# selbouhaddani/PPLS

Measured on AMD Instinct MI355X. Metric: EM iterations/sec + log-lik rel-err vs CPU ref, n=1e6 p=q=2000 r=5, higher is better.
Workload: dtype f64

## Files before the change

### include/ppls_debug.h

```cpp
#ifndef PPLS_AMD_PPLS_DEBUG_H
#define PPLS_AMD_PPLS_DEBUG_H

#include "ppls.h"

#ifdef __cplusplus
extern "C" {
#endif

int ppls_sweep_timing(ppls_ctx* ctx, double* total_ms, int64_t* launches, int reset);
int ppls_sweep_balance(ppls_ctx* ctx, double* w8, int64_t* bounds, int cap, int* n_bounds);
int ppls_comm_info(ppls_ctx* ctx, int* nranks, int* rank, double* allreduce_ms, int64_t* allreduce_calls,
                   int reset);
int ppls_xprod_info(ppls_ctx* ctx, int r, int* ready, int64_t* bytes_per_pass, double* flops, int* rows_per_wave);
int ppls_xprod_setup_times(ppls_ctx* ctx, double* gram_ms, double* allreduce_ms, double* total_ms);
int ppls_xprod_tile_timing(ppls_ctx* ctx, int reps, double* ms);
int ppls_xprod_stats(ppls_ctx* ctx, const ppls_theta* th, int r, double* stats);
int ppls_sweep_info(ppls_ctx* ctx, int r, int64_t* bytes_per_sweep, int* variant, int* grid);
int ppls_sweep_kernel(ppls_ctx* ctx, int r, char* buf, int len);
int ppls_gram_int8(ppls_ctx* ctx, int which, double* G, int* nmod, int* L, double* ms);
int ppls_gram_shifts(ppls_ctx* ctx, int* shift, int P, int* count);
int ppls_oz_residue_host(double x, int shift, int l, int* r);
int ppls_oz_crt_host(const int* r, int nmod, double* out);
int ppls_oz_modulus(int l);
int ppls_gram_info(ppls_ctx* ctx, int* int8_used, int* nmod, int* L, double* ms);
int ppls_meta_info(ppls_ctx* ctx, int* path);
int ppls_gram(ppls_ctx* ctx, int xory, int nsplit, double* G, double* ms);
int ppls_spd_inverse(ppls_ctx* ctx, const double* A, int p, int a, int method, double* out, int* info, double* ms);
int ppls_philox4x32_10(ppls_ctx* ctx, const uint32_t* ctr, int64_t count, uint64_t key, uint32_t* out);

#define PPLS_FTRACE_LEN 48
int ppls_finalize_trace(ppls_ctx* ctx, int64_t* stamps, double* tick_ns);
#define PPLS_STRACE_MAX_WG 4096
int ppls_sweep_trace(ppls_ctx* ctx, int64_t* stamps, int cap, int* n, double* tick_ns);
int ppls_cv_timing(ppls_ctx* ctx, double* out6, int reset);

int ppls_xprod_get(ppls_ctx* ctx, double* S, int* P, int* ldx);

int ppls_scale_timing(ppls_ctx* ctx, double* ms3, double* bytes3);

// ... 7 lines not shown
```

### ppls_amd/_lib.py

```python
from __future__ import annotations

import ctypes as ct
import os

import numpy as np

_HERE = os.path.dirname(os.path.abspath(__file__))
LIB_PATH = os.path.join(_HERE, "libppls_amd.so")

PPLS_OK = 0
PPLS_ORTH_SVD = 0
PPLS_ORTH_QR = 1
PPLS_LAYOUT_COLMAJOR = 0
PPLS_LAYOUT_ROWMAJOR = 1

_dp = ct.POINTER(ct.c_double)


class PplsTheta(ct.Structure):
    _fields_ = [("W", _dp), ("C", _dp), ("B", _dp), ("sigT", _dp),
                ("sigE", ct.c_double), ("sigF", ct.c_double), ("sigH", ct.c_double)]


class PplsExpect(ct.Structure):
# ... 81 lines not shown
    "ppls_comm_info": (ct.c_int, [ct.c_void_p, ct.POINTER(ct.c_int), ct.POINTER(ct.c_int), _dp,
                                  ct.POINTER(ct.c_int64), ct.c_int]),
    "ppls_finalize_trace": (ct.c_int, [ct.c_void_p, ct.POINTER(ct.c_int64), _dp]),
    "ppls_sweep_trace": (ct.c_int, [ct.c_void_p, ct.POINTER(ct.c_int64), ct.c_int, ct.POINTER(ct.c_int), _dp]),
    "ppls_sweep_info": (ct.c_int, [ct.c_void_p, ct.c_int, ct.POINTER(ct.c_int64), ct.POINTER(ct.c_int),
                                   ct.POINTER(ct.c_int)]),
    "ppls_sweep_kernel": (ct.c_int, [ct.c_void_p, ct.c_int, ct.c_char_p, ct.c_int]),
    "ppls_meta_info": (ct.c_int, [ct.c_void_p, ct.POINTER(ct.c_int)]),
    "ppls_gram_int8": (ct.c_int, [ct.c_void_p, ct.c_int, _dp, ct.POINTER(ct.c_int), ct.POINTER(ct.c_int), _dp]),
    "ppls_oz_residue_host": (ct.c_int, [ct.c_double, ct.c_int, ct.c_int, ct.POINTER(ct.c_int)]),
    "ppls_oz_crt_host": (ct.c_int, [ct.POINTER(ct.c_int), ct.c_int, _dp]),
    "ppls_oz_modulus": (ct.c_int, [ct.c_int]),
    "ppls_gram_info": (ct.c_int, [ct.c_void_p, ct.POINTER(ct.c_int), ct.POINTER(ct.c_int), ct.POINTER(ct.c_int),
                                  _dp]),
    "ppls_gram_shifts": (ct.c_int, [ct.c_void_p, ct.POINTER(ct.c_int), ct.c_int, ct.POINTER(ct.c_int)]),
    "ppls_finalize_host": (ct.c_int, [_dp, _dp, _dp, ct.c_double, ct.c_double, ct.c_double, ct.c_int,
                                      ct.c_int, ct.c_int, ct.POINTER(PplsTheta), ct.c_int,
                                      ct.POINTER(PplsTheta), ct.POINTER(PplsExpect), _dp]),
    "ppls_mu_coefficients": (ct.c_int, [ct.POINTER(PplsTheta), ct.c_int, _dp]),
    "ppls_set_data_from": (ct.c_int, [ct.c_void_p, ct.c_void_p, _i64p, ct.c_int64, ct.c_int64]),
    "ppls_xprod_downdate": (ct.c_int, [ct.c_void_p, ct.c_void_p, _i64p, ct.c_int64]),
    "ppls_predict": (ct.c_int, [ct.c_void_p, _dp, _dp, _dp, ct.c_int, ct.c_int, _dp, ct.c_int64, ct.c_int, _dp]),
    "ppls_heldout_sse": (ct.c_int, [ct.c_void_p, _dp, _dp, _dp, ct.c_int, _i64p, ct.c_int64, _dp]),
    "ppls_cv_ppls": (ct.c_int, [ct.c_void_p, ct.c_int, ct.c_int, ct.POINTER(ct.c_int32), _i64p, ct.c_int,
                                ct.c_double, ct.c_int, ct.POINTER(PplsTheta), _dp, ct.POINTER(ct.c_int)]),
    "ppls_cv_timing": (ct.c_int, [ct.c_void_p, _dp, ct.c_int]),
    "ppls_scale_data": (ct.c_int, [ct.c_void_p, ct.c_int, ct.c_int]),
    "ppls_get_scaling": (ct.c_int, [ct.c_void_p, _dp, _dp]),
    "ppls_scale_timing": (ct.c_int, [ct.c_void_p, _dp, _dp]),
    "ppls_xprod_get": (ct.c_int, [ct.c_void_p, _dp, ct.POINTER(ct.c_int), ct.POINTER(ct.c_int)]),
# ... 113 lines not shown
```

### ppls_amd/api.py

```python
from __future__ import annotations

import ctypes as ct
import itertools
import math
import time
import warnings

import numpy as np

from . import _lib
from ._lib import Expect, PplsError, Theta, dptr


def pop_rows(pop_sizes, row0, n_local):
    sizes = np.asarray(pop_sizes, dtype=np.int64)
    ends = np.cumsum(sizes)
    begins = ends - sizes
    lo, hi = int(row0), int(row0) + int(n_local)
    local = np.clip(np.minimum(ends, hi) - np.maximum(begins, lo), 0, None).astype(np.int64)
    return np.ascontiguousarray(local), np.ascontiguousarray(sizes)


class Context:

# ... 419 lines not shown
        nm, L, ms = ct.c_int(), ct.c_int(), np.zeros(4)
        self._chk(self._L.ppls_gram_int8(self.h, int(which), dptr(G), ct.byref(nm), ct.byref(L), dptr(ms)))
        return G, dict(nmod=nm.value, L=L.value, ms=ms.tolist(), shift=self.gram_shifts())

    def gram_shifts(self):
        k = ct.c_int()
        self._chk(self._L.ppls_gram_shifts(self.h, None, 0, ct.byref(k)))
        out = (ct.c_int * max(k.value, 1))()
        self._chk(self._L.ppls_gram_shifts(self.h, out, k.value, ct.byref(k)))
        return np.array(out[:k.value], dtype=np.int64)

    def gram_info(self):
        u, nm, L, ms = ct.c_int(), ct.c_int(), ct.c_int(), np.zeros(4)
        self._chk(self._L.ppls_gram_info(self.h, ct.byref(u), ct.byref(nm), ct.byref(L), dptr(ms)))
        return dict(int8=bool(u.value), nmod=nm.value, L=L.value, ms=ms.tolist())

    def spd_inverse(self, A, method=1):
        A = np.asarray(A, dtype=np.float64)
        one = A.ndim == 2
        A3 = A[None] if one else A
        a, p = A3.shape[0], A3.shape[1]
        Af = np.ascontiguousarray(np.transpose(A3, (0, 2, 1)))
        out = np.empty_like(Af)
        info = (ct.c_int * a)()
        ms = ct.c_double()
        self._chk(self._L.ppls_spd_inverse(self.h, dptr(Af), int(p), int(a), int(method), dptr(out), info,
                                            ct.byref(ms)))
        inv = np.transpose(out, (0, 2, 1))
        return (inv[0] if one else inv), np.array(list(info)), ms.value

# ... 969 lines not shown
```

### ppls_amd/csrc/ppls_capi.cpp

```cpp
#include <hip/hip_runtime.h>
#include <rccl/rccl.h>
#include <rocblas/rocblas.h>
#include <rocsolver/rocsolver.h>

#include <algorithm>
#include <chrono>
#include <cmath>
#include <cstdarg>
#include <cstdio>
#include <cstring>
#include <string>
#include <utility>
#include <vector>

#include "../../include/ppls.h"
#include "../../include/ppls_debug.h"
#include "ppls_kernels.h"
#include "ppls_math.h"
#include "ppls_cv.h"
#include "ppls_scale.h"
#include "ppls_cvstream.h"
#include "ppls_stream.h"
#include "ppls_xprod.h"

// ... 61 lines not shown
  int bal_grid = -1;
  double bal_w[8] = {1, 1, 1, 1, 1, 1, 1, 1};
  int64_t* bal_bounds = nullptr;
  double* coefs = nullptr;
  double* scratch = nullptr;
  size_t scratch_bytes = 0;
  int* stop_d = nullptr;
  int* stop_mirror = nullptr;
  int* stop_mirror_dev = nullptr;
  const int* sweep_stop = nullptr;
  double stop_atol = 0.0;
  int em_r = 0, em_cur = 0, em_iter = 0;
  bool em_active = false;
  int xprod = 0;
  int xprod_rw = 0;
  int gram_int8 = 0;
  int oz_used = 0, oz_nmod = 0, oz_L = 0;
  std::vector<int> oz_shift;
  double oz_ms[4] = {0, 0, 0, 0};
  int8_t* oz_planes = nullptr;
  uint8_t* oz_res = nullptr;
  size_t oz_planes_len = 0, oz_res_len = 0;
  bool xp_ready = false;
  bool xp_active = false;
  bool xp_pending_gram = false;
  int xprod_fuse = 1;
  bool xp_explicit = false;
  int meta_path = 0;
  int meta_device = 1;
  int vorth = 8;
  double* xp_S = nullptr;
// ... 605 lines not shown
  if (!part_in) dfree(part);
  if (e != hipSuccess) return fail(c, PPLS_E_HIP, "MFMA Gram: %s", hipGetErrorString(e));
  return PPLS_OK;
}

bool oz_held(const ppls_ctx* c) { return c->oz_planes || c->oz_res; }

void oz_free(ppls_ctx* c) {
  dfree(c->oz_planes);
  dfree(c->oz_res);
  c->oz_planes = nullptr;
  c->oz_res = nullptr;
  c->oz_planes_len = c->oz_res_len = 0;
}

int gram_run_oz(ppls_ctx* c, const GramShape& g, int64_t n, double* G, float* ms) {
  const int P = g.p, Pp = (P + 255) / 256 * 256;
  const int64_t nkb = (n + PPLS_OZ_KS - 1) / PPLS_OZ_KS;
  const int dtype = c->dtype;
  struct Bufs {
    double* part = nullptr;
    double* st = nullptr;
    int* shift = nullptr;
    hipEvent_t ev[5] = {nullptr, nullptr, nullptr, nullptr, nullptr};
    ~Bufs() {
      dfree(part); dfree(st); dfree(shift);
      for (auto e : ev) if (e) (void)hipEventDestroy(e);
    }
  } b;
  int rc;
  const int chunks = (int)std::max<int64_t>(1, std::min<int64_t>(256, n / 2048));
  if ((rc = dalloc(c, &b.part, (size_t)chunks * 2 * Pp)) || (rc = dalloc(c, &b.st, (size_t)2 * Pp)) ||
      (rc = dalloc(c, &b.shift, (size_t)Pp)))
    return rc;
  for (auto& e : b.ev) HIPCHK(c, hipEventCreate(&e));
  HIPCHK(c, hipEventRecord(b.ev[0], c->stream));
  HIPCHK(c, ppls_launch_oz_colstats(g.X, g.ldx, g.xcols, g.xreal, g.Y, g.ldy, g.yreal, dtype, Pp, n, chunks, b.part,
                                    b.st, c->stream));
  std::vector<double> st((size_t)2 * Pp);
  HIPCHK(c, hipMemcpyAsync(st.data(), b.st, sizeof(double) * st.size(), hipMemcpyDeviceToHost, c->stream));
  HIPCHK(c, hipStreamSynchronize(c->stream));
  auto live = [&](int j) { return j < g.xreal || (j >= g.xcols && j - g.xcols < g.yreal); };
  int L = 55;
  std::vector<int> shift((size_t)Pp, 0);
  double qmax = 0.0;
  for (int j = 0; j < P; ++j) {
    if (!live(j) || !(st[(size_t)j] > 0.0)) continue;
    int ex = 0;
    (void)std::frexp(st[(size_t)j], &ex);
    const double cj = std::max(1.0, std::ldexp(1.0, ex) * std::sqrt((double)n / st[(size_t)Pp + j]));
    const int Lj = 53 + (int)std::ceil(std::log2(cj)) + 2;
    L = std::max(L, Lj);
    shift[(size_t)j] = Lj - ex;
    const double q = std::ldexp(std::sqrt(st[(size_t)Pp + j]), Lj - ex) + 0.5 * std::sqrt((double)n);
    qmax = std::max(qmax, q * q);
  }
  c->oz_L = L;
  c->oz_shift.assign(shift.begin(), shift.begin() + P);
  if (L > 62) return 1;
  const double need = std::log2(std::max(qmax, 1.0)) + 1.0 + 1e-7;
  double bits = 0.0;
  int nmod = 0;
  while (nmod < PPLS_OZ_MAXMOD && bits < need) bits += std::log2((double)ppls_oz_modulus(nmod++));
  if (bits < need) return 1;
  nmod = std::max(nmod, 12);
  c->oz_nmod = nmod;
  const int T = Pp / 256, ntiles = T * (T + 1) / 2, nsplit = ppls_oz_splits(nkb);
  const int64_t pstride = nkb * Pp * PPLS_OZ_KS;
  const size_t need_planes = (size_t)nmod * pstride, need_res = (size_t)nmod * nsplit * ntiles * 65536;
  if (need_planes > c->oz_planes_len || need_res > c->oz_res_len) {
    HIPCHK(c, hipStreamSynchronize(c->stream));
    oz_free(c);
    size_t fr = 0, tot = 0;
    if (hipMemGetInfo(&fr, &tot) != hipSuccess) return 1;
    const double want = (double)need_planes + (double)need_res;
    if (want > (double)fr - std::max(1073741824.0, 0.05 * (double)fr)) return 1;
    if (dalloc(c, &c->oz_planes, need_planes) || dalloc(c, &c->oz_res, need_res)) {
      c->err.clear();
      oz_free(c);
      return 1;
    }
    c->oz_planes_len = need_planes;
    c->oz_res_len = need_res;
  }
  int8_t* planes = c->oz_planes;
  uint8_t* res = c->oz_res;
  HIPCHK(c, hipMemcpyAsync(b.shift, shift.data(), sizeof(int) * Pp, hipMemcpyHostToDevice, c->stream));
  HIPCHK(c, ppls_launch_oz_residues(g.X, g.ldx, g.xcols, g.xreal, g.Y, g.ldy, g.yreal, dtype, Pp, n, nkb, b.shift,
                                    nmod, planes, pstride, c->stream));
  HIPCHK(c, hipEventRecord(b.ev[1], c->stream));
  HIPCHK(c, ppls_launch_oz_syrk(planes, pstride, Pp, nkb, nmod, res, c->stream));
  HIPCHK(c, hipEventRecord(b.ev[2], c->stream));
  HIPCHK(c, ppls_launch_oz_finish(res, nmod, nsplit, Pp, g.xcols, g.xreal, g.yreal, P, b.shift, G, c->stream));
  HIPCHK(c, hipEventRecord(b.ev[3], c->stream));
  HIPCHK(c, hipStreamSynchronize(c->stream));
  float t01 = 0.f, t12 = 0.f, t23 = 0.f, t03 = 0.f;
  HIPCHK(c, hipEventElapsedTime(&t01, b.ev[0], b.ev[1]));
  HIPCHK(c, hipEventElapsedTime(&t12, b.ev[1], b.ev[2]));
  HIPCHK(c, hipEventElapsedTime(&t23, b.ev[2], b.ev[3]));
  HIPCHK(c, hipEventElapsedTime(&t03, b.ev[0], b.ev[3]));
  c->oz_ms[0] = t01;
  c->oz_ms[1] = t12;
  c->oz_ms[2] = t23;
  c->oz_ms[3] = t03;
  if (ms) *ms = t03;
  return PPLS_OK;
}

int gram_run_s(ppls_ctx* c, const GramShape& g, int64_t n, double* G, float* ms, double* part) {
  c->oz_used = 0;
  if (c->gram_int8) {
    const int rc = gram_run_oz(c, g, n, G, ms);
    if (rc == PPLS_OK) {
      c->oz_used = 1;
      return PPLS_OK;
    }
    if (rc < 0) return rc;
  }
  return gram_run(c, g, n, 0, G, ms, part);
}

int xprod_setup(ppls_ctx* c);
bool xprod_choose(ppls_ctx* c, int max_steps, int r);

int64_t xprod_rows(const ppls_ctx* c) { return (c->n_total + c->nranks - 1) / c->nranks; }

double xprod_bytes(ppls_ctx* c) {
  const GramShape g = gram_shape(c, true, 0);
  const double PP = (double)g.p * g.p;
  return 8.0 * PP + 8.0 * (double)ppls_gram_part_doubles(g.p, gram_nsplit(c, g, xprod_rows(c), 0)) +
         16.0 * g.p * PPLS_RMAX;
}
// ... 63 lines not shown
  return PPLS_OK;
}

bool xprod_choose(ppls_ctx* c, int max_steps, int r) {
  if (c->st_state == 2) return true;
  if (c->xprod == 0) return false;
  if (c->xprod == 1) return true;
  if (!c->xp_ready && xprod_bytes(c) > c->mem_free_min - std::max(1073741824.0, 0.05 * c->mem_free_min))
    return false;
  const double P = (double)(c->ldx + c->ldy);
  const double n = (double)((c->n_total + c->nranks - 1) / c->nranks);
  const double esz = c->dtype ? 4.0 : 8.0;
  const bool split = c->sweep_mode != 3 && !c->dtype && ppls_split_supported(r, c->ldx, c->ldy) > 0;
  const double t_sweep = (split ? 1.0 : 2.0) * esz * n * P / 6.5e12 + 5e-6;
  const double t_pass = 8.0 * P * P / 6.5e12 + 5e-6;
  const double gram_rate = c->gram_int8 ? 1.0e14 : 55e12;
  const double t_setup = c->xp_ready ? 0.0 : n * P * P / gram_rate + (c->nranks > 1 ? 16.0 * P * P / 100e9 : 0.0);
  return ((double)max_steps + 1.0) * (t_sweep - t_pass) > t_setup;
}

int xprod_stats(ppls_ctx* c, int r, int slot, bool fuse) {
  int rc;
  const int P = c->ldx + c->ldy;
  if (!c->xp_ready && (rc = xprod_setup(c))) return rc;
  if (!c->xp_M) {
    if ((rc = dalloc(c, &c->xp_M, (size_t)P * 2 * PPLS_RMAX))) return rc;
  }
  hipEvent_t e0, e1;
  if ((rc = timing_pair(c, &e0, &e1))) return rc;
  if (e0) HIPCHK(c, hipEventRecord(e0, c->stream));
  const int rw = ppls_xprod_tile_rows(P, r, c->xprod_rw, c->num_cus);
// ... 56 lines not shown
  c->st_fq.clear();
  c->st_fq_len.clear();
  c->st_cap = c->st_cm_len = c->st_part_len = c->st_colpart_len = c->st_gbuf_len = 0;
  c->st_state = 0;
  c->st_failed = false;
}

void fold_free(ppls_ctx* c) {
  dfree(c->st_fS);
  c->st_nfolds = 0;
  c->st_sel = -1;
  c->st_fN.clear();
  c->st_fmean_h.clear();
}

void xprod_free(ppls_ctx* c) {
  if (c->st_state) {
    stream_release(c);
    c->have_data = false;
    c->em_active = false;
  }
  c->xp_ready = false;
  c->xp_explicit = false;
  c->xp_active = false;
  dfree(c->xp_S);
  dfree(c->xp_M);
  fold_free(c);
}

int compute_ssq(ppls_ctx* c) {
  int rc;
  xprod_free(c);

  const int nb = 1024;
  const int nred = 2 + c->nranks;
  if ((rc = dalloc(c, &c->scratch, (size_t)nb + nred))) return rc;
  HIPCHK(c, hipMemsetAsync(c->ssq, 0, 2 * sizeof(double), c->stream));
  if (c->n_local > 0 && c->dtype) {
    HIPCHK(c, ppls_launch_sumsq_f32((const float*)c->X, c->n_local * c->ldx, c->scratch, nb, c->ssq, c->stream));
    HIPCHK(c, ppls_launch_sumsq_f32((const float*)c->Y, c->n_local * c->ldy, c->scratch, nb, c->ssq + 1, c->stream));
  } else if (c->n_local > 0) {
    HIPCHK(c, ppls_launch_sumsq(c->X, c->n_local * c->ldx, c->scratch, nb, c->ssq, 0, c->stream));
// ... 290 lines not shown
      c->have_data = false;
    }
  } else if (!strcmp(key, "nt")) {
    if (value < -1 || value > 1) return fail(c, PPLS_E_ARG, "nt must be -1 (auto), 0 or 1");
    c->nt_loads = (int)value;
  } else if (!strcmp(key, "xprod")) {
    if (value < -1 || value > 1) return fail(c, PPLS_E_ARG, "xprod must be -1 (auto), 0 (stream X, Y) or 1 (cross-products)");
    if (value == 0 && c->em_active && c->xp_active && c->st_state != 2) {
      c->em_active = false;
      c->xp_active = false;
    }
    const int was = c->xprod;
    c->xprod = (int)value;
    if (value == 0 && was != 0 && !c->xp_explicit && c->st_state == 0) {
      HIPCHK(c, hipStreamSynchronize(c->stream));
      xprod_free(c);
    }
  } else if (!strcmp(key, "meta_device")) {
    c->meta_device = value ? 1 : 0;
  } else if (!strcmp(key, "vorth")) {
    if (value < 1 || value > 255) return fail(c, PPLS_E_ARG, "vorth must be in [1, 255]");
    c->vorth = (int)value;
  } else if (!strcmp(key, "xprod_fuse")) {
    c->xprod_fuse = value ? 1 : 0;
  } else if (!strcmp(key, "var_chol")) {
    if (value < 0 || value > 2) return fail(c, PPLS_E_ARG, "var_chol must be 0 (LU), 1 (Cholesky) or 2 (rocSOLVER Cholesky)");
    c->var_chol = (int)value;
  } else if (!strcmp(key, "gram_int8")) {
    if (value < 0 || value > 1) return fail(c, PPLS_E_ARG, "gram_int8 must be 0 (fp64 MFMA Gram) or 1 (int8 CRT form)");
    if ((int)value != c->gram_int8) {
      c->gram_int8 = (int)value;
      if (c->xp_ready && !c->xp_explicit) {
        dfree(c->xp_S);
        c->xp_ready = false;
      }
      if (!c->gram_int8) {
        HIPCHK(c, hipStreamSynchronize(c->stream));
        oz_free(c);
      }
    }
  } else if (!strcmp(key, "xprod_rw")) {
    if (value != 0 && value != 1 && value != 2 && value != 4 && value != 8)
      return fail(c, PPLS_E_ARG, "xprod_rw must be 0, 1, 2, 4 or 8");
    c->xprod_rw = (int)value;
  } else if (!strcmp(key, "timing")) {
    if (value < 0) return fail(c, PPLS_E_ARG, "timing must be >= 0");
    c->timing = (int)value;
    c->sweep_count = 0;
  } else {
    return fail(c, PPLS_E_ARG, "unknown option '%s'", key);
  }
  return PPLS_OK;
}

void ppls_shard_range(int64_t n_total, int nranks, int rank, int64_t* row0, int64_t* n_local) {
// ... 1620 lines not shown
  if (!c->have_data) return fail(c, PPLS_E_STATE, "no data");
  HIPCHK(c, hipSetDevice(c->device));
  const bool was = c->xp_ready;
  int rc;
  if ((rc = xprod_setup(c))) return rc;
  c->xp_explicit = true;
  if (ms) *ms = was ? 0.0 : c->xp_setup_ms;
  if (total_ms) *total_ms = was ? 0.0 : c->xp_setup_total_ms;
  return PPLS_OK;
}

int ppls_xprod_release(ppls_ctx* c) {
  if (!c) return PPLS_E_ARG;
  HIPCHK(c, hipSetDevice(c->device));
  HIPCHK(c, hipStreamSynchronize(c->stream));
  xprod_free(c);
  return PPLS_OK;
}

int ppls_xprod_get(ppls_ctx* c, double* S, int* P, int* ldx) {
  if (!c) return PPLS_E_ARG;
  if (!c->have_data || !c->xp_ready || !c->xp_S) return fail(c, PPLS_E_STATE, "no cross-products S are ready");
  const int PP = c->ldx + c->ldy;
  if (P) *P = PP;
  if (ldx) *ldx = c->ldx;
  if (S) {
    HIPCHK(c, hipSetDevice(c->device));
    HIPCHK(c, hipStreamSynchronize(c->stream));
    HIPCHK(c, hipMemcpy(S, c->xp_S, sizeof(double) * PP * PP, hipMemcpyDeviceToHost));
  }
  return PPLS_OK;
// ... 156 lines not shown

int ppls_gram_shifts(ppls_ctx* c, int* shift, int P, int* count) {
  if (!c) return PPLS_E_ARG;
  const int k = (int)c->oz_shift.size();
  if (count) *count = k;
  if (shift) for (int j = 0; j < std::min(P, k); ++j) shift[j] = c->oz_shift[(size_t)j];
  return PPLS_OK;
}

int ppls_gram_info(ppls_ctx* c, int* int8_used, int* nmod, int* L, double* ms) {
  if (!c) return PPLS_E_ARG;
  if (int8_used) *int8_used = c->oz_used;
  if (nmod) *nmod = c->oz_nmod;
  if (L) *L = c->oz_L;
  if (ms) for (int k = 0; k < 4; ++k) ms[k] = c->oz_ms[k];
  return PPLS_OK;
}

int ppls_meta_info(ppls_ctx* c, int* path) {
  if (!c || !path) return PPLS_E_ARG;
  *path = c->meta_path;
  return PPLS_OK;
}

int ppls_sweep_kernel(ppls_ctx* c, int r, char* buf, int len) {
  if (!c || !buf || len < 1) return PPLS_E_ARG;
  if (r < 1 || r > PPLS_RMAX) return fail(c, PPLS_E_ARG, "bad r");
  PplsSweepArgs a;
  const int plan = sweep_plan(c, r, &a);
  const int nt = c->nt_loads > 0 ||
// ... 417 lines not shown
      return fail(c, PPLS_E_ARG, "fold %d: %zu local rows, %lld over all ranks", f, in_fold[(size_t)f].size(), (long long)fold_total[f]);
  for (int k = 0; k < nfolds * a; ++k)
    if (!init[k].W || !init[k].C || !init[k].B || !init[k].sigT) return fail(c, PPLS_E_ARG, "init[%d] has NULL fields", k);
  HIPCHK(c, hipSetDevice(c->device));
  int rc;
  if (!c->cv_train && (rc = ppls_ctx_create(c->device, &c->cv_train))) return fail(c, rc, "could not create the training context");
  ppls_ctx* t = c->cv_train;
  t->xprod = c->xprod;
  t->xprod_rw = c->xprod_rw;
  t->xprod_fuse = c->xprod_fuse;
  if (t->gram_int8 && !c->gram_int8) {
    HIPCHK(c, hipStreamSynchronize(t->stream));
    oz_free(t);
  }
  t->gram_int8 = c->gram_int8;
  t->ldpad = c->ldpad;
  t->sweep_mode = c->sweep_mode;
  t->grid_opt = c->grid_opt;
  t->nt_loads = c->nt_loads;
  t->reducer = c->reducer;
  t->reducer_user = c->reducer_user;
  t->comm = c->comm;
  t->nranks = c->nranks;
  t->rank = c->rank;
  const int p = c->p, q = c->q;
  std::vector<double> W((size_t)p * a), C((size_t)q * a), B((size_t)a), sig((size_t)4 * a), sse((size_t)a);
  std::vector<int64_t> train;
  for (int f = 0; f < nfolds; ++f) {
    const std::vector<int64_t>& out = in_fold[(size_t)f];
    train.clear();
// ... 917 lines not shown
```

### ppls_amd/csrc/ppls_kernels.h

```cpp
#pragma once

#include <hip/hip_runtime.h>
#include <stdint.h>

#include "ppls_math.h"

#define PPLS_SWEEP_SLOTS 4
#define PPLS_FUSED_RMAX 8

struct PplsSweepArgs {
  const double* X;
  const double* Y;
  int64_t n_local;
  int p, q;
  int ldx, ldy;
  const double* Wp;
  const double* Cp;
  const PplsScalars* sc;
  double* part;
  int64_t part_ld;
  double* mu;
  int write_mu;
  int r;
  int ns;
// ... 151 lines not shown
                              double k2, double bstar, double s4, double N, double* M, double* sst_exp,
                              double* sst_star, hipStream_t st);
hipError_t ppls_launch_negdiag(double* M, int p, double* se, hipStream_t st);
hipError_t ppls_launch_negate(double* M, int64_t len, hipStream_t st);
hipError_t ppls_launch_symdiag(double* M, int p, double* se, hipStream_t st);
int64_t ppls_spd_inverse_work(int p, int a);
hipError_t ppls_spd_inverse_batched(double* A, int p, int a, double* work, int* info, hipStream_t st);
hipError_t ppls_launch_to_colmajor(const double* src, int64_t n, int p, int ld, double* dst,
                                   hipStream_t st);
int ppls_oz_modulus(int l);
hipError_t ppls_launch_oz_colstats(const void* X, int ldx, int xcols, int xreal, const void* Y, int ldy, int yreal,
                                   int f32, int Pp, int64_t n, int chunks, double* part, double* out, hipStream_t st);
hipError_t ppls_launch_oz_residues(const void* X, int ldx, int xcols, int xreal, const void* Y, int ldy, int yreal,
                                   int f32, int Pp, int64_t n, int64_t nkb, const int* shift, int nmod, int8_t* planes,
                                   int64_t pstride, hipStream_t st);
int ppls_oz_splits(int64_t nkb);
hipError_t ppls_launch_oz_syrk(const int8_t* planes, int64_t pstride, int Pp, int64_t nkb, int nmod, uint8_t* part,
                               hipStream_t st);
hipError_t ppls_launch_oz_finish(const uint8_t* part, int nmod, int nsplit, int Pp, int xcols, int xreal, int yreal,
                                 int P, const int* shift, double* G, hipStream_t st);
}
```

### ppls_amd/csrc/ppls_ozaki.hip

```cpp
#include <hip/hip_runtime.h>
#include <stdint.h>

#include <type_traits>

#include "ppls_device.h"
#include "ppls_kernels.h"

namespace {

constexpr int OZ_TT = 256;
constexpr int OZ_KS = PPLS_OZ_KS;
constexpr int OZ_PANEL = OZ_TT * OZ_KS;
constexpr int OZ_SPLIT_STAGES = 1024;

__host__ __device__ constexpr int oz_mod(int l) {
  switch (l) {
    case 0: return 256;  case 1: return 255;  case 2: return 253;  case 3: return 251;  case 4: return 247;
    case 5: return 241;  case 6: return 239;  case 7: return 233;  case 8: return 229;  case 9: return 227;
    case 10: return 223; case 11: return 217; case 12: return 211; case 13: return 199; case 14: return 197;
    case 15: return 193; case 16: return 191; case 17: return 181; case 18: return 179; case 19: return 173;
    default: return 1;
  }
}

// ... 138 lines not shown
    uint32_t w[4] = {0, 0, 0, 0};
#pragma unroll
    for (int k = 0; k < 16; ++k)
      w[k >> 2] |= ((uint32_t)oz_residue21(la[k], lb[k], lc[k], m, k42, k21, bias) & 255u) << (8 * (k & 3));
    *(v4i*)(dst + (int64_t)l * pstride) = v4i{(int)w[0], (int)w[1], (int)w[2], (int)w[3]};
  }
}

__device__ __forceinline__ int oz_lds_off(int c, int q) { return c * OZ_KS + ((q ^ ((c >> 2) & 3)) << 4); }

typedef __attribute__((address_space(3))) void* oz_lptr;

template <int A>
__global__ __launch_bounds__((A & 4) ? 512 : 256, 1) void ppls_oz_syrk_kernel(
    const int8_t* __restrict__ planes, int64_t pstride, int Pp, int64_t nkb, int nmod, int nsplit, int ntiles,
    uint8_t* __restrict__ out) {
  constexpr int NWV = (A & 4) ? 8 : 4;
  constexpr int CT = 256 / (NWV / 2);
  constexpr int NJ = CT / 32;
  constexpr int NU = 16 / NWV;
  constexpr int NC = 2 * NU;
  __shared__ __attribute__((aligned(16))) int8_t ring[4 * 2 * OZ_PANEL];
  const int b = blockIdx.x, nb = gridDim.x;
  const int it = (b & 7) * (nb >> 3) + (b >> 3);
  if (it >= nmod * nsplit * ntiles) return;
  const int l = it / (nsplit * ntiles), rem = it - l * nsplit * ntiles;
  const int sp = rem / ntiles, t = rem - sp * ntiles;
  const int64_t s0 = (int64_t)sp * OZ_SPLIT_STAGES;
  const int64_t s1 = s0 + OZ_SPLIT_STAGES < nkb ? s0 + OZ_SPLIT_STAGES : nkb;
  const int m = oz_mod(l);
  int I, J;
// ... 57 lines not shown
      for (int j = 0; j < NJ; ++j) acc[i][j] = __builtin_amdgcn_mfma_i32_32x32x32_i8(a1[i], b1[j], acc[i][j], 0, 0, 0);
      if (4 + i < NC) dma(nq, sn, 4 + i);
    }
  };
#pragma unroll
  for (int k = 0; k < 3; ++k)
#pragma unroll
    for (int g = 0; g < NC; ++g) dma(k, last(s0 + k), g);
  for (int64_t s = s0; s < s1; s += 4) {
    stage(0, s);
    if (s + 1 < s1) stage(1, s + 1);
    if (s + 2 < s1) stage(2, s + 2);
    if (s + 3 < s1) stage(3, s + 3);
  }
  ppls_wait_vmcnt(0);
#pragma unroll
  for (int i = 0; i < 4; ++i)
#pragma unroll
    for (int j = 0; j < NJ; ++j)
#pragma unroll
      for (int r = 0; r < 16; ++r) {
        const int v = acc[i][j][r] % m;
        acc[i][j][r] = v < 0 ? v + m : v;
      }
  if (idle) return;
  uint8_t* o = out + (int64_t)it * OZ_TT * OZ_TT;
#pragma unroll
  for (int i = 0; i < 4; ++i)
#pragma unroll
    for (int j = 0; j < NJ; ++j) {
      const int col = CT * wj + 32 * j + (lane & 31);
#pragma unroll
      for (int gq = 0; gq < 4; ++gq) {
        const int row = 128 * wi + 32 * i + 8 * gq + 4 * h;
        const uint32_t v = (uint32_t)acc[i][j][4 * gq] | ((uint32_t)acc[i][j][4 * gq + 1] << 8) |
                           ((uint32_t)acc[i][j][4 * gq + 2] << 16) | ((uint32_t)acc[i][j][4 * gq + 3] << 24);
        *(uint32_t*)(o + (int64_t)col * OZ_TT + row) = v;
      }
    }
}

namespace {

template <int NMOD>
__host__ __device__ __forceinline__ double oz_crt(const int (&r)[NMOD], const OzTab& tab) {
  int d[NMOD];
#pragma unroll
  for (int l = 0; l < NMOD; ++l) {
    const int m = oz_mod(l);
    int t = r[l];
#pragma unroll
    for (int k = 0; k < l; ++k) {
      t = t - d[k] + 2 * m;
      t = (t * tab.inv[l][k]) % m;
// ... 129 lines not shown
  const int64_t rpc = (n + chunks - 1) / chunks;
  const dim3 grid((unsigned)((Pp + 255) / 256), (unsigned)chunks);
  if (f32)
    hipLaunchKernelGGL(ppls_oz_colstats_kernel<float>, grid, dim3(256), 0, st, (const float*)X, ldx, (const float*)Y,
                       ldy, g, Pp, n, rpc, part);
  else
    hipLaunchKernelGGL(ppls_oz_colstats_kernel<double>, grid, dim3(256), 0, st, (const double*)X, ldx,
                       (const double*)Y, ldy, g, Pp, n, rpc, part);
  hipLaunchKernelGGL(ppls_oz_colstats_finish_kernel, dim3((unsigned)((Pp + 255) / 256)), dim3(256), 0, st, part, chunks,
                     Pp, out);
  return hipGetLastError();
}

#define OZ_NMOD_CASES(X) X(12) X(13) X(14) X(15) X(16) X(17) X(18) X(19) X(20)

hipError_t ppls_launch_oz_residues(const void* X, int ldx, int xcols, int xreal, const void* Y, int ldy, int yreal,
                                   int f32, int Pp, int64_t n, int64_t nkb, const int* shift, int nmod, int8_t* planes,
                                   int64_t pstride, hipStream_t st) {
  const OzCols g{xreal, xcols, yreal};
  const dim3 grid((unsigned)((Pp + 63) / 64), (unsigned)nkb);
#define OZ_RES(N)                                                                                               \
  case N:                                                                                                       \
    if (f32)                                                                                                    \
      hipLaunchKernelGGL((ppls_oz_residue_kernel<float, N>), grid, dim3(256), 0, st, (const float*)X, ldx,      \
                         (const float*)Y, ldy, g, Pp, n, shift, planes, pstride);                               \
    else                                                                                                        \
      hipLaunchKernelGGL((ppls_oz_residue_kernel<double, N>), grid, dim3(256), 0, st, (const double*)X, ldx,    \
                         (const double*)Y, ldy, g, Pp, n, shift, planes, pstride);                              \
    break;
  switch (nmod) {
    OZ_NMOD_CASES(OZ_RES)
    default: return hipErrorInvalidValue;
  }
#undef OZ_RES
  return hipGetLastError();
}

int ppls_oz_splits(int64_t nkb) { return (int)((nkb + OZ_SPLIT_STAGES - 1) / OZ_SPLIT_STAGES); }

hipError_t ppls_launch_oz_syrk_v(int variant, const int8_t* planes, int64_t pstride, int Pp, int64_t nkb, int nmod,
                                 uint8_t* part, hipStream_t st) {
  const int T = Pp / OZ_TT, ntiles = T * (T + 1) / 2, nsplit = ppls_oz_splits(nkb);
  const int64_t items = (int64_t)nmod * nsplit * ntiles;
  const int64_t grid = (items + 7) / 8 * 8;
  if (grid > 0x7fffffff) return hipErrorInvalidValue;
#define OZ_SYRK(AV)                                                                                             \
  case AV:                                                                                                      \
    hipLaunchKernelGGL(ppls_oz_syrk_kernel<AV>, dim3((unsigned)grid), dim3(((AV) & 4) ? 512 : 256), 0, st, planes, \
                       pstride, Pp, nkb, nmod, nsplit, ntiles, part);                                           \
    break;
  switch (variant) {
    OZ_SYRK(0)
#ifdef OZ_LAB
    OZ_SYRK(1) OZ_SYRK(2) OZ_SYRK(4) OZ_SYRK(5) OZ_SYRK(6)
#endif
    default: return hipErrorInvalidValue;
  }
#undef OZ_SYRK
  return hipGetLastError();
}

hipError_t ppls_launch_oz_syrk(const int8_t* planes, int64_t pstride, int Pp, int64_t nkb, int nmod, uint8_t* part,
                               hipStream_t st) {
  return ppls_launch_oz_syrk_v(0, planes, pstride, Pp, nkb, nmod, part, st);
}

hipError_t ppls_launch_oz_finish(const uint8_t* part, int nmod, int nsplit, int Pp, int xcols, int xreal, int yreal,
                                 int P, const int* shift, double* G, hipStream_t st) {
  const OzCols g{xreal, xcols, yreal};
  const int T = Pp / OZ_TT, ntiles = T * (T + 1) / 2;
  const dim3 grid((unsigned)ntiles, (unsigned)(OZ_TT / 16));
#define OZ_FIN(N)                                                                                               \
  case N:                                                                                                       \
    hipLaunchKernelGGL((ppls_oz_finish_kernel<N>), grid, dim3(256), 0, st, part, nsplit, ntiles, g, P, shift, G); \
// ... 11 lines not shown
```

Before: 206.9.

## Auto-enable chunked int8 Ozaki Gram with bounded workspace and accumulating syrk

Makes the int8 CRT (Ozaki) Gram path the default whenever n·Pp² passes a threshold, in place of the fp64 MFMA Gram. Rows are processed in chunks: the residue planes for each row chunk are built and reduced by a syrk that adds modularly into persistent per-split output tiles. This bounds the plane workspace by a memory cap and by a split count sized to the CU count. Allocation failures now fall back to the fp64 path instead of erroring. The aim is to cut the one-time cross-product setup cost; the trade-off is more launches, read-modify-write of the residue tiles, and more workspace memory that is now kept alive by default.

```diff
diff --git a/include/ppls_debug.h b/include/ppls_debug.h
--- a/include/ppls_debug.h
+++ b/include/ppls_debug.h
@@ -23,6 +23,7 @@
 int ppls_oz_crt_host(const int* r, int nmod, double* out);
 int ppls_oz_modulus(int l);
 int ppls_gram_info(ppls_ctx* ctx, int* int8_used, int* nmod, int* L, double* ms);
+int ppls_gram_workspace(ppls_ctx* ctx, int64_t* bytes, int* splits_per_chunk, int* num_cus);
 int ppls_meta_info(ppls_ctx* ctx, int* path);
 int ppls_gram(ppls_ctx* ctx, int xory, int nsplit, double* G, double* ms);
 int ppls_spd_inverse(ppls_ctx* ctx, const double* A, int p, int a, int method, double* out, int* info, double* ms);
diff --git a/ppls_amd/_lib.py b/ppls_amd/_lib.py
--- a/ppls_amd/_lib.py
+++ b/ppls_amd/_lib.py
@@ -119,6 +119,8 @@
     "ppls_gram_info": (ct.c_int, [ct.c_void_p, ct.POINTER(ct.c_int), ct.POINTER(ct.c_int), ct.POINTER(ct.c_int),
                                   _dp]),
     "ppls_gram_shifts": (ct.c_int, [ct.c_void_p, ct.POINTER(ct.c_int), ct.c_int, ct.POINTER(ct.c_int)]),
+    "ppls_gram_workspace": (ct.c_int, [ct.c_void_p, ct.POINTER(ct.c_int64), ct.POINTER(ct.c_int),
+                                       ct.POINTER(ct.c_int)]),
     "ppls_finalize_host": (ct.c_int, [_dp, _dp, _dp, ct.c_double, ct.c_double, ct.c_double, ct.c_int,
                                       ct.c_int, ct.c_int, ct.POINTER(PplsTheta), ct.c_int,
                                       ct.POINTER(PplsTheta), ct.POINTER(PplsExpect), _dp]),
diff --git a/ppls_amd/api.py b/ppls_amd/api.py
--- a/ppls_amd/api.py
+++ b/ppls_amd/api.py
@@ -457,6 +457,11 @@
         u, nm, L, ms = ct.c_int(), ct.c_int(), ct.c_int(), np.zeros(4)
         self._chk(self._L.ppls_gram_info(self.h, ct.byref(u), ct.byref(nm), ct.byref(L), dptr(ms)))
         return dict(int8=bool(u.value), nmod=nm.value, L=L.value, ms=ms.tolist())
+
+    def gram_workspace(self):
+        b, s, cu = ct.c_int64(), ct.c_int(), ct.c_int()
+        self._chk(self._L.ppls_gram_workspace(self.h, ct.byref(b), ct.byref(s), ct.byref(cu)))
+        return dict(bytes=b.value, splits_per_chunk=s.value, num_cus=cu.value)
 
     def spd_inverse(self, A, method=1):
         A = np.asarray(A, dtype=np.float64)
diff --git a/ppls_amd/csrc/ppls_capi.cpp b/ppls_amd/csrc/ppls_capi.cpp
--- a/ppls_amd/csrc/ppls_capi.cpp
+++ b/ppls_amd/csrc/ppls_capi.cpp
@@ -99,7 +99,11 @@
   bool em_active = false;
   int xprod = 0;
   int xprod_rw = 0;
-  int gram_int8 = 0;
+  int gram_int8 = -1;
+  double oz_auto_min = 4e12;
+  int oz_chunk_opt = 0;
+  double oz_mem_cap = 0.0;
+  int oz_chunk_splits = 0;
   int oz_used = 0, oz_nmod = 0, oz_L = 0;
   std::vector<int> oz_shift;
   double oz_ms[4] = {0, 0, 0, 0};
@@ -735,6 +739,17 @@
   c->oz_planes_len = c->oz_res_len = 0;
 }
 
+int oz_chunk_rule(const ppls_ctx* c, int nmod, int ntiles) {
+  const int64_t per_split = (int64_t)nmod * ntiles, want = (int64_t)32 * c->num_cus;
+  return (int)std::min<int64_t>(63, std::max<int64_t>(1, (want + per_split - 1) / per_split));
+}
+
+bool oz_wanted(const ppls_ctx* c, int p, int64_t n) {
+  if (c->gram_int8 >= 0) return c->gram_int8 == 1;
+  const double Pp = (double)((p + 255) / 256 * 256);
+  return (double)n * Pp * Pp >= c->oz_auto_min;
+}
+
 int gram_run_oz(ppls_ctx* c, const GramShape& g, int64_t n, double* G, float* ms) {
   const int P = g.p, Pp = (P + 255) / 256 * 256;
   const int64_t nkb = (n + PPLS_OZ_KS - 1) / PPLS_OZ_KS;
@@ -743,24 +758,36 @@
     double* part = nullptr;
     double* st = nullptr;
     int* shift = nullptr;
-    hipEvent_t ev[5] = {nullptr, nullptr, nullptr, nullptr, nullptr};
+    std::vector<hipEvent_t> ev;
     ~Bufs() {
       dfree(part); dfree(st); dfree(shift);
       for (auto e : ev) if (e) (void)hipEventDestroy(e);
     }
   } b;
-  int rc;
-  const int chunks = (int)std::max<int64_t>(1, std::min<int64_t>(256, n / 2048));
-  if ((rc = dalloc(c, &b.part, (size_t)chunks * 2 * Pp)) || (rc = dalloc(c, &b.st, (size_t)2 * Pp)) ||
-      (rc = dalloc(c, &b.shift, (size_t)Pp)))
-    return rc;
-  for (auto& e : b.ev) HIPCHK(c, hipEventCreate(&e));
-  HIPCHK(c, hipEventRecord(b.ev[0], c->stream));
-  HIPCHK(c, ppls_launch_oz_colstats(g.X, g.ldx, g.xcols, g.xreal, g.Y, g.ldy, g.yreal, dtype, Pp, n, chunks, b.part,
-                                    b.st, c->stream));
+  auto decline = [&]() {
+    (void)hipGetLastError();
+    c->err.clear();
+    return 1;
+  };
+#define OZTRY(call)                                \
+  do {                                             \
+    if ((call) != hipSuccess) return decline();    \
+  } while (0)
+  const int64_t total_splits = ppls_oz_splits(nkb);
+  const int stat_chunks = (int)std::max<int64_t>(1, std::min<int64_t>(256, n / 2048));
+  if (dalloc(c, &b.part, (size_t)stat_chunks * 2 * Pp) || dalloc(c, &b.st, (size_t)2 * Pp) || dalloc(c, &b.shift, (size_t)Pp))
+    return decline();
+  {
+    hipEvent_t e0 = nullptr;
+    OZTRY(hipEventCreate(&e0));
+    b.ev.push_back(e0);
+  }
+  OZTRY(hipEventRecord(b.ev[0], c->stream));
+  OZTRY(ppls_launch_oz_colstats(g.X, g.ldx, g.xcols, g.xreal, g.Y, g.ldy, g.yreal, dtype, Pp, n, stat_chunks, b.part, b.st,
+                                c->stream));
   std::vector<double> st((size_t)2 * Pp);
-  HIPCHK(c, hipMemcpyAsync(st.data(), b.st, sizeof(double) * st.size(), hipMemcpyDeviceToHost, c->stream));
-  HIPCHK(c, hipStreamSynchronize(c->stream));
+  OZTRY(hipMemcpyAsync(st.data(), b.st, sizeof(double) * st.size(), hipMemcpyDeviceToHost, c->stream));
+  OZTRY(hipStreamSynchronize(c->stream));
   auto live = [&](int j) { return j < g.xreal || (j >= g.xcols && j - g.xcols < g.yreal); };
   int L = 55;
   std::vector<int> shift((size_t)Pp, 0);
@@ -786,57 +813,88 @@
   if (bits < need) return 1;
   nmod = std::max(nmod, 12);
   c->oz_nmod = nmod;
-  const int T = Pp / 256, ntiles = T * (T + 1) / 2, nsplit = ppls_oz_splits(nkb);
-  const int64_t pstride = nkb * Pp * PPLS_OZ_KS;
-  const size_t need_planes = (size_t)nmod * pstride, need_res = (size_t)nmod * nsplit * ntiles * 65536;
+  const int T = Pp / 256, ntiles = T * (T + 1) / 2;
+  int cs = (int)std::min<int64_t>(total_splits, c->oz_chunk_opt > 0 ? c->oz_chunk_opt : oz_chunk_rule(c, nmod, ntiles));
+  auto stages_of = [&](int k) { return std::min<int64_t>((int64_t)k * 1024, nkb); };
+  auto bytes_of = [&](int k) {
+    return (double)nmod * (double)stages_of(k) * Pp * PPLS_OZ_KS + (double)nmod * k * ntiles * 65536.0;
+  };
+  size_t need_planes = (size_t)nmod * stages_of(cs) * Pp * PPLS_OZ_KS, need_res = (size_t)nmod * cs * ntiles * 65536;
+  const bool grow = need_planes > c->oz_planes_len || need_res > c->oz_res_len;
+  if (grow || c->oz_mem_cap > 0.0) {
+    size_t fr = 0, tot = 0;
+    if (grow) {
+      OZTRY(hipStreamSynchronize(c->stream));
+      oz_free(c);
+    }
+    if (hipMemGetInfo(&fr, &tot) != hipSuccess) return decline();
+    double room = (double)fr + (double)c->oz_planes_len + (double)c->oz_res_len;
+    if (c->oz_mem_cap > 0.0) room = std::min(room, c->oz_mem_cap);
+    room -= std::max(1073741824.0, 0.05 * room);
+    while (cs > 1 && bytes_of(cs) > room) --cs;
+    if (bytes_of(cs) > room) return 1;
+    need_planes = (size_t)nmod * stages_of(cs) * Pp * PPLS_OZ_KS;
+    need_res = (size_t)nmod * cs * ntiles * 65536;
+  }
   if (need_planes > c->oz_planes_len || need_res > c->oz_res_len) {
-    HIPCHK(c, hipStreamSynchronize(c->stream));
-    oz_free(c);
-    size_t fr = 0, tot = 0;
-    if (hipMemGetInfo(&fr, &tot) != hipSuccess) return 1;
-    const double want = (double)need_planes + (double)need_res;
-    if (want > (double)fr - std::max(1073741824.0, 0.05 * (double)fr)) return 1;
     if (dalloc(c, &c->oz_planes, need_planes) || dalloc(c, &c->oz_res, need_res)) {
-      c->err.clear();
       oz_free(c);
-      return 1;
+      return decline();
     }
     c->oz_planes_len = need_planes;
     c->oz_res_len = need_res;
   }
+  const int64_t cstages = stages_of(cs), crows = cstages * PPLS_OZ_KS;
+  const int64_t pstride = cstages * Pp * PPLS_OZ_KS;
+  const int nchunks = (int)((nkb + cstages - 1) / cstages);
+  c->oz_chunk_splits = cs;
   int8_t* planes = c->oz_planes;
   uint8_t* res = c->oz_res;
-  HIPCHK(c, hipMemcpyAsync(b.shift, shift.data(), sizeof(int) * Pp, hipMemcpyHostToDevice, c->stream));
-  HIPCHK(c, ppls_launch_oz_residues(g.X, g.ldx, g.xcols, g.xreal, g.Y, g.ldy, g.yreal, dtype, Pp, n, nkb, b.shift,
-                                    nmod, planes, pstride, c->stream));
-  HIPCHK(c, hipEventRecord(b.ev[1], c->stream));
-  HIPCHK(c, ppls_launch_oz_syrk(planes, pstride, Pp, nkb, nmod, res, c->stream));
-  HIPCHK(c, hipEventRecord(b.ev[2], c->stream));
-  HIPCHK(c, ppls_launch_oz_finish(res, nmod, nsplit, Pp, g.xcols, g.xreal, g.yreal, P, b.shift, G, c->stream));
-  HIPCHK(c, hipEventRecord(b.ev[3], c->stream));
-  HIPCHK(c, hipStreamSynchronize(c->stream));
-  float t01 = 0.f, t12 = 0.f, t23 = 0.f, t03 = 0.f;
-  HIPCHK(c, hipEventElapsedTime(&t01, b.ev[0], b.ev[1]));
-  HIPCHK(c, hipEventElapsedTime(&t12, b.ev[1], b.ev[2]));
-  HIPCHK(c, hipEventElapsedTime(&t23, b.ev[2], b.ev[3]));
-  HIPCHK(c, hipEventElapsedTime(&t03, b.ev[0], b.ev[3]));
-  c->oz_ms[0] = t01;
-  c->oz_ms[1] = t12;
-  c->oz_ms[2] = t23;
-  c->oz_ms[3] = t03;
-  if (ms) *ms = t03;
+  for (int k = 0; k < 2 * nchunks + 1; ++k) {
+    hipEvent_t e = nullptr;
+    OZTRY(hipEventCreate(&e));
+    b.ev.push_back(e);
+  }
+  OZTRY(hipMemcpyAsync(b.shift, shift.data(), sizeof(int) * Pp, hipMemcpyHostToDevice, c->stream));
+  for (int k = 0; k < nchunks; ++k) {
+    const int64_t row0 = (int64_t)k * crows, rows = std::min<int64_t>(crows, n - row0);
+    const int64_t kstages = (rows + PPLS_OZ_KS - 1) / PPLS_OZ_KS;
+    OZTRY(ppls_launch_oz_residues_rows(g.X, g.ldx, g.xcols, g.xreal, g.Y, g.ldy, g.yreal, dtype, Pp, row0, rows, kstages,
+                                       b.shift, nmod, planes, pstride, c->stream));
+    OZTRY(hipEventRecord(b.ev[(size_t)1 + 2 * k], c->stream));
+    OZTRY(ppls_launch_oz_syrk_chunk(0, planes, pstride, Pp, kstages, nmod, cs, k > 0 ? 1 : 0, res, c->stream));
+    OZTRY(hipEventRecord(b.ev[(size_t)2 + 2 * k], c->stream));
+  }
+  OZTRY(ppls_launch_oz_finish(res, nmod, cs, Pp, g.xcols, g.xreal, g.yreal, P, b.shift, G, c->stream));
+  OZTRY(hipEventRecord(b.ev.back(), c->stream));
+  OZTRY(hipStreamSynchronize(c->stream));
+  double t_res = 0.0, t_syrk = 0.0;
+  float t = 0.f;
+  for (int k = 0; k < nchunks; ++k) {
+    OZTRY(hipEventElapsedTime(&t, b.ev[(size_t)2 * k], b.ev[(size_t)2 * k + 1]));
+    t_res += t;
+    OZTRY(hipEventElapsedTime(&t, b.ev[(size_t)2 * k + 1], b.ev[(size_t)2 * k + 2]));
+    t_syrk += t;
+  }
+  c->oz_ms[0] = t_res;
+  c->oz_ms[1] = t_syrk;
+  OZTRY(hipEventElapsedTime(&t, b.ev[b.ev.size() - 2], b.ev.back()));
+  c->oz_ms[2] = t;
+  OZTRY(hipEventElapsedTime(&t, b.ev[0], b.ev.back()));
+  c->oz_ms[3] = t;
+  if (ms) *ms = t;
+#undef OZTRY
   return PPLS_OK;
 }
 
 int gram_run_s(ppls_ctx* c, const GramShape& g, int64_t n, double* G, float* ms, double* part) {
   c->oz_used = 0;
-  if (c->gram_int8) {
+  if (oz_wanted(c, g.p, n)) {
     const int rc = gram_run_oz(c, g, n, G, ms);
     if (rc == PPLS_OK) {
       c->oz_used = 1;
       return PPLS_OK;
     }
-    if (rc < 0) return rc;
   }
   return gram_run(c, g, n, 0, G, ms, part);
 }
@@ -930,7 +988,7 @@
   const bool split = c->sweep_mode != 3 && !c->dtype && ppls_split_supported(r, c->ldx, c->ldy) > 0;
   const double t_sweep = (split ? 1.0 : 2.0) * esz * n * P / 6.5e12 + 5e-6;
   const double t_pass = 8.0 * P * P / 6.5e12 + 5e-6;
-  const double gram_rate = c->gram_int8 ? 1.0e14 : 55e12;
+  const double gram_rate = oz_wanted(c, c->ldx + c->ldy, (int64_t)n) ? 1.0e14 : 55e12;
   const double t_setup = c->xp_ready ? 0.0 : n * P * P / gram_rate + (c->nranks > 1 ? 16.0 * P * P / 100e9 : 0.0);
   return ((double)max_steps + 1.0) * (t_sweep - t_pass) > t_setup;
 }
@@ -1017,7 +1075,7 @@
   c->st_fmean_h.clear();
 }
 
-void xprod_free(ppls_ctx* c) {
+void xprod_free(ppls_ctx* c, bool release_ws = false) {
   if (c->st_state) {
     stream_release(c);
     c->have_data = false;
@@ -1029,6 +1087,10 @@
   dfree(c->xp_S);
   dfree(c->xp_M);
   fold_free(c);
+  if (release_ws && c->gram_int8 < 0 && oz_held(c)) {
+    if (c->stream) (void)hipStreamSynchronize(c->stream);
+    oz_free(c);
+  }
 }
 
 int compute_ssq(ppls_ctx* c) {
@@ -1349,7 +1411,7 @@
     c->xprod = (int)value;
     if (value == 0 && was != 0 && !c->xp_explicit && c->st_state == 0) {
       HIPCHK(c, hipStreamSynchronize(c->stream));
-      xprod_free(c);
+      xprod_free(c, true);
     }
   } else if (!strcmp(key, "meta_device")) {
     c->meta_device = value ? 1 : 0;
@@ -1362,7 +1424,8 @@
     if (value < 0 || value > 2) return fail(c, PPLS_E_ARG, "var_chol must be 0 (LU), 1 (Cholesky) or 2 (rocSOLVER Cholesky)");
     c->var_chol = (int)value;
   } else if (!strcmp(key, "gram_int8")) {
-    if (value < 0 || value > 1) return fail(c, PPLS_E_ARG, "gram_int8 must be 0 (fp64 MFMA Gram) or 1 (int8 CRT form)");
+    if (value < -1 || value > 1)
+      return fail(c, PPLS_E_ARG, "gram_int8 must be -1 (auto), 0 (fp64 MFMA Gram) or 1 (int8 CRT form)");
     if ((int)value != c->gram_int8) {
       c->gram_int8 = (int)value;
       if (c->xp_ready && !c->xp_explicit) {
@@ -1374,6 +1437,15 @@
         oz_free(c);
       }
     }
+  } else if (!strcmp(key, "gram_int8_chunk")) {
+    if (value < 0 || value > 63) return fail(c, PPLS_E_ARG, "gram_int8_chunk must be 0 (auto) or 1 .. 63 splits per row chunk");
+    c->oz_chunk_opt = (int)value;
+  } else if (!strcmp(key, "gram_int8_min")) {
+    if (value < 0) return fail(c, PPLS_E_ARG, "gram_int8_min must be >= 0");
+    c->oz_auto_min = (double)value;
+  } else if (!strcmp(key, "gram_int8_mem_cap")) {
+    if (value < 0) return fail(c, PPLS_E_ARG, "gram_int8_mem_cap must be >= 0 bytes (0: no cap)");
+    c->oz_mem_cap = (double)value;
   } else if (!strcmp(key, "xprod_rw")) {
     if (value != 0 && value != 1 && value != 2 && value != 4 && value != 8)
       return fail(c, PPLS_E_ARG, "xprod_rw must be 0, 1, 2, 4 or 8");
@@ -3024,7 +3096,7 @@
   if (!c) return PPLS_E_ARG;
   HIPCHK(c, hipSetDevice(c->device));
   HIPCHK(c, hipStreamSynchronize(c->stream));
-  xprod_free(c);
+  xprod_free(c, true);
   return PPLS_OK;
 }
 
@@ -3211,6 +3283,14 @@
   if (nmod) *nmod = c->oz_nmod;
   if (L) *L = c->oz_L;
   if (ms) for (int k = 0; k < 4; ++k) ms[k] = c->oz_ms[k];
+  return PPLS_OK;
+}
+
+int ppls_gram_workspace(ppls_ctx* c, int64_t* bytes, int* splits_per_chunk, int* num_cus) {
+  if (!c) return PPLS_E_ARG;
+  if (bytes) *bytes = (int64_t)(c->oz_planes_len + c->oz_res_len);
+  if (splits_per_chunk) *splits_per_chunk = c->oz_chunk_splits;
+  if (num_cus) *num_cus = c->num_cus;
   return PPLS_OK;
 }
 
@@ -3658,6 +3738,9 @@
     oz_free(t);
   }
   t->gram_int8 = c->gram_int8;
+  t->oz_auto_min = c->oz_auto_min;
+  t->oz_chunk_opt = c->oz_chunk_opt;
+  t->oz_mem_cap = c->oz_mem_cap;
   t->ldpad = c->ldpad;
   t->sweep_mode = c->sweep_mode;
   t->grid_opt = c->grid_opt;
diff --git a/ppls_amd/csrc/ppls_kernels.h b/ppls_amd/csrc/ppls_kernels.h
--- a/ppls_amd/csrc/ppls_kernels.h
+++ b/ppls_amd/csrc/ppls_kernels.h
@@ -189,7 +189,12 @@
 hipError_t ppls_launch_oz_residues(const void* X, int ldx, int xcols, int xreal, const void* Y, int ldy, int yreal,
                                    int f32, int Pp, int64_t n, int64_t nkb, const int* shift, int nmod, int8_t* planes,
                                    int64_t pstride, hipStream_t st);
+hipError_t ppls_launch_oz_residues_rows(const void* X, int ldx, int xcols, int xreal, const void* Y, int ldy, int yreal,
+                                        int f32, int Pp, int64_t row0, int64_t n, int64_t nkb, const int* shift, int nmod,
+                                        int8_t* planes, int64_t pstride, hipStream_t st);
 int ppls_oz_splits(int64_t nkb);
+hipError_t ppls_launch_oz_syrk_chunk(int variant, const int8_t* planes, int64_t pstride, int Pp, int64_t nkb, int nmod,
+                                     int osplit, int accum, uint8_t* part, hipStream_t st);
 hipError_t ppls_launch_oz_syrk(const int8_t* planes, int64_t pstride, int Pp, int64_t nkb, int nmod, uint8_t* part,
                                hipStream_t st);
 hipError_t ppls_launch_oz_finish(const uint8_t* part, int nmod, int nsplit, int Pp, int xcols, int xreal, int yreal,
diff --git a/ppls_amd/csrc/ppls_ozaki.hip b/ppls_amd/csrc/ppls_ozaki.hip
--- a/ppls_amd/csrc/ppls_ozaki.hip
+++ b/ppls_amd/csrc/ppls_ozaki.hip
@@ -176,7 +176,7 @@
 template <int A>
 __global__ __launch_bounds__((A & 4) ? 512 : 256, 1) void ppls_oz_syrk_kernel(
     const int8_t* __restrict__ planes, int64_t pstride, int Pp, int64_t nkb, int nmod, int nsplit, int ntiles,
-    uint8_t* __restrict__ out) {
+    int osplit, int accum, uint8_t* __restrict__ out) {
   constexpr int NWV = (A & 4) ? 8 : 4;
   constexpr int CT = 256 / (NWV / 2);
   constexpr int NJ = CT / 32;
@@ -264,30 +264,48 @@
     if (s + 3 < s1) stage(3, s + 3);
   }
   ppls_wait_vmcnt(0);
-#pragma unroll
-  for (int i = 0; i < 4; ++i)
-#pragma unroll
-    for (int j = 0; j < NJ; ++j)
+  if (idle) return;
+  uint8_t* o = out + (((int64_t)l * osplit + sp) * ntiles + t) * OZ_TT * OZ_TT;
+  const bool add = accum != 0;
+  const uint8_t* po = o;
+  asm volatile("" : "+v"(po));
+  auto off = [&](int b, int gq) {
+    const int i = b / NJ, j = b % NJ;
+    return (CT * wj + 32 * j + (lane & 31)) * OZ_TT + 128 * wi + 32 * i + 8 * gq + 4 * h;
+  };
+  uint32_t pv[4] = {0, 0, 0, 0}, nx[4] = {0, 0, 0, 0};
+  if (add) {
+#pragma unroll
+    for (int gq = 0; gq < 4; ++gq) pv[gq] = *(const uint32_t*)(po + off(0, gq));
+  }
+#pragma unroll
+  for (int b = 0; b < 4 * NJ; ++b) {
+    const int i = b / NJ, j = b % NJ;
+    if (add && b + 1 < 4 * NJ) {
+#pragma unroll
+      for (int gq = 0; gq < 4; ++gq) nx[gq] = *(const uint32_t*)(po + off(b + 1, gq));
+    }
+#pragma unroll
+    for (int r = 0; r < 16; ++r) {
+      const int v = acc[i][j][r] % m;
+      acc[i][j][r] = v < 0 ? v + m : v;
+    }
+    if (add) {
 #pragma unroll
       for (int r = 0; r < 16; ++r) {
-        const int v = acc[i][j][r] % m;
-        acc[i][j][r] = v < 0 ? v + m : v;
+        const int v = acc[i][j][r] + (int)((pv[r >> 2] >> (8 * (r & 3))) & 255u);
+        acc[i][j][r] = v >= m ? v - m : v;
       }
-  if (idle) return;
-  uint8_t* o = out + (int64_t)it * OZ_TT * OZ_TT;
-#pragma unroll
-  for (int i = 0; i < 4; ++i)
-#pragma unroll
-    for (int j = 0; j < NJ; ++j) {
-      const int col = CT * wj + 32 * j + (lane & 31);
-#pragma unroll
-      for (int gq = 0; gq < 4; ++gq) {
-        const int row = 128 * wi + 32 * i + 8 * gq + 4 * h;
-        const uint32_t v = (uint32_t)acc[i][j][4 * gq] | ((uint32_t)acc[i][j][4 * gq + 1] << 8) |
-                           ((uint32_t)acc[i][j][4 * gq + 2] << 16) | ((uint32_t)acc[i][j][4 * gq + 3] << 24);
-        *(uint32_t*)(o + (int64_t)col * OZ_TT + row) = v;
-      }
-    }
+    }
+#pragma unroll
+    for (int gq = 0; gq < 4; ++gq) {
+      const uint32_t v = (uint32_t)acc[i][j][4 * gq] | ((uint32_t)acc[i][j][4 * gq + 1] << 8) |
+                         ((uint32_t)acc[i][j][4 * gq + 2] << 16) | ((uint32_t)acc[i][j][4 * gq + 3] << 24);
+      *(uint32_t*)(o + off(b, gq)) = v;
+    }
+#pragma unroll
+    for (int gq = 0; gq < 4; ++gq) pv[gq] = nx[gq];
+  }
 }
 
 namespace {
@@ -447,6 +465,15 @@
 
 #define OZ_NMOD_CASES(X) X(12) X(13) X(14) X(15) X(16) X(17) X(18) X(19) X(20)
 
+hipError_t ppls_launch_oz_residues_rows(const void* X, int ldx, int xcols, int xreal, const void* Y, int ldy, int yreal,
+                                        int f32, int Pp, int64_t row0, int64_t n, int64_t nkb, const int* shift, int nmod,
+                                        int8_t* planes, int64_t pstride, hipStream_t st) {
+  const int64_t es = f32 ? 4 : 8;
+  return ppls_launch_oz_residues(X ? (const char*)X + row0 * ldx * es : nullptr, ldx, xcols, xreal,
+                                 Y ? (const char*)Y + row0 * ldy * es : nullptr, ldy, yreal, f32, Pp, n, nkb, shift, nmod,
+                                 planes, pstride, st);
+}
+
 hipError_t ppls_launch_oz_residues(const void* X, int ldx, int xcols, int xreal, const void* Y, int ldy, int yreal,
                                    int f32, int Pp, int64_t n, int64_t nkb, const int* shift, int nmod, int8_t* planes,
                                    int64_t pstride, hipStream_t st) {
@@ -471,16 +498,17 @@
 
 int ppls_oz_splits(int64_t nkb) { return (int)((nkb + OZ_SPLIT_STAGES - 1) / OZ_SPLIT_STAGES); }
 
-hipError_t ppls_launch_oz_syrk_v(int variant, const int8_t* planes, int64_t pstride, int Pp, int64_t nkb, int nmod,
-                                 uint8_t* part, hipStream_t st) {
+hipError_t ppls_launch_oz_syrk_chunk(int variant, const int8_t* planes, int64_t pstride, int Pp, int64_t nkb, int nmod,
+                                     int osplit, int accum, uint8_t* part, hipStream_t st) {
   const int T = Pp / OZ_TT, ntiles = T * (T + 1) / 2, nsplit = ppls_oz_splits(nkb);
+  if (osplit < nsplit) return hipErrorInvalidValue;
   const int64_t items = (int64_t)nmod * nsplit * ntiles;
   const int64_t grid = (items + 7) / 8 * 8;
   if (grid > 0x7fffffff) return hipErrorInvalidValue;
 #define OZ_SYRK(AV)                                                                                             \
   case AV:                                                                                                      \
     hipLaunchKernelGGL(ppls_oz_syrk_kernel<AV>, dim3((unsigned)grid), dim3(((AV) & 4) ? 512 : 256), 0, st, planes, \
-                       pstride, Pp, nkb, nmod, nsplit, ntiles, part);                                           \
+                       pstride, Pp, nkb, nmod, nsplit, ntiles, osplit, accum, part);                            \
     break;
   switch (variant) {
     OZ_SYRK(0)
@@ -491,6 +519,11 @@
   }
 #undef OZ_SYRK
   return hipGetLastError();
+}
+
+hipError_t ppls_launch_oz_syrk_v(int variant, const int8_t* planes, int64_t pstride, int Pp, int64_t nkb, int nmod,
+                                 uint8_t* part, hipStream_t st) {
+  return ppls_launch_oz_syrk_chunk(variant, planes, pstride, Pp, nkb, nmod, ppls_oz_splits(nkb), 0, part, st);
 }
 
 hipError_t ppls_launch_oz_syrk(const int8_t* planes, int64_t pstride, int Pp, int64_t nkb, int nmod, uint8_t* part,
```

Result: no change. 205.9 (-0.5%).
